# nucypher/TFHE.jl

Measured on AMD Instinct MI355X. Metric: bootstrapped gates/sec (whole node), N=1024, higher is better.
Workload: dtype int32 torus / f64 transform; 1 GPU; batch of 4096 independent gate_nand() bootstraps per GPU, tfhe_parameters_80 (n=500, N=1024, k=1, l=2, Bg=2^10, ks t=8, base 2^2); inputs=resident in HBM, launch=one process

## Files before the change

tfhe.jl_amd/csrc/engine.hpp:

```cpp
#pragma once
#include <hip/hip_runtime.h>

#include <algorithm>
#include <atomic>
#include <cstdarg>
#include <cstdio>
#include <cstring>
#include <new>
#include <string>
#include <thread>
#include <vector>

#include "../../include/tfhe_mi355x.h"
#include "experiment.hpp"
#include "br_core.hpp"

using namespace tfhe;

#include "kernels_blind_rotate.hpp"
#include "kernels_anyn.hpp"
#include "kernels_n512.hpp"
#include "kernels_keyswitch.hpp"

struct ErrBuf {
    char s[512] = {0};
    const char *c_str() const { return s; }
    void set(const char *msg) { snprintf(s, sizeof s, "%s", msg ? msg : ""); }
    ErrBuf &operator=(const char *msg) { set(msg); return *this; }
    void format(const char *fmt, ...) __attribute__((format(printf, 2, 3)))
    {
        va_list ap;
        va_start(ap, fmt);
        vsnprintf(s, sizeof s, fmt, ap);
        va_end(ap);
    }
};
extern thread_local ErrBuf g_create_error;

struct DevBuf {
    void *p = nullptr;
    size_t cap = 0;
    hipError_t reserve(size_t bytes)
    {
        if (bytes <= cap) return hipSuccess;
        if (p) (void)hipFree(p);
        p = nullptr; cap = 0;
        size_t want = bytes + bytes / 4 + 256;
        hipError_t e = hipMalloc(&p, want);
        if (e == hipSuccess) cap = want;
        return e;
    }
    void release() { if (p) (void)hipFree(p); p = nullptr; cap = 0; }
};

struct PairXfer {
    static constexpr int kSlots = 4;
    struct Slot {
        DevBuf out, idx_src;
        DevBuf in, idx_dst;
        int32_t *h_idx = nullptr; size_t h_idx_cap = 0;
        void *h_rows = nullptr; size_t h_rows_cap = 0;
        hipEvent_t ready = nullptr;
        hipEvent_t taken = nullptr;
        bool pending = false;
    } slot[kSlots];
    unsigned next = 0;
};

struct KsKey {
    int mode = 0;
    int parties = 1;
    int kN = 0;
    void *p = nullptr;
    size_t per_party = 0;
    int stride = 0;
    int wtiles = 0;
};
inline void release(KsKey &k)
{
    if (k.p) (void)hipFree(k.p);
    k = KsKey{};
}

struct tfhe_ctx {
    tfhe_params P{};
    int device = 0;
    ErrBuf err;
    std::vector<tfhe_ctx *> kids;
    std::vector<uint8_t> kid_ran;

    hipStream_t stream = nullptr;
    static constexpr int kTimingSlots = 33;
    hipEvent_t evring[kTimingSlots][4] = {};
    hipEvent_t *ev = evring[0];
    int64_t timed_calls = 0;
    hipEvent_t done_ev = nullptr;
    bool done_pending = false;
    bool timing_valid = false;
    bool own_pending = false;
    int64_t last_rotations = 0;
    std::string last_kernel;
    int ks_slices_large = 2;
    int ks_variant = 4;
    int64_t br_small = 1024;
    int br_prio_pct = 90;
    int br_general = 0;
    int br_split = 1;
    int timing_events = 1;
    int br_rt_l = 0;
    int64_t br_tiny = -2;

    cplx *d_tables = nullptr;
    Tables T{};
    Gadget g{};
    cplx *d_anyn_tab = nullptr;
    int br_anyn = 0;
    int anyn_spec = -1;
    bool anyn() const
    {
        if (br_anyn) return true;
        if (P.parties > 1) return P.N != kN || P.parties > 8 || P.bs_l > 8;
        if (n512()) return false;
        return (P.N != kN && P.N != 2048) || P.k > 4;
    }
    bool n512() const { return !br_anyn && P.parties == 1 && P.N == 512 && P.k == 1; }

    cplx *d_bk = nullptr;       size_t bk_polys = 0;
    KsKey ks;
    bool have_bk = false;
    bool have_ks() const { return ks.mode != 0 && ks.parties == 1; }
    cplx *d_mk_bk = nullptr;
    int mk_parties = 0;
    bool have_mk_bk = false;
    bool have_mk_ks() const { return ks.mode != 0 && ks.parties > 1; }

    int32_t *d_wires = nullptr; int64_t num_wires = 0;
    int wires_parties = 0;
    size_t wire_words() const { return wires_parties ? (size_t)wires_parties * P.n + 1 : (size_t)P.n + 1; }

    DevBuf bara, ext, map, io[4], diag, abar, mk_acc, spec;
    DevBuf tv, tv_index;
    DevBuf tv_bodies, tv_ext;
    cplx *d_tgsw = nullptr;        int64_t tgsw_count = 0;
    DevBuf lvl_ws[2], lvl_data, lvl_spec;
    cplx *d_mk_tgsw = nullptr;     int64_t mk_tgsw_count = 0;
    int32_t *d_mk_tgsw_party = nullptr;
    size_t diag_rows = 0;
    bool mk_force_general = false;
    int n2048_rw = 0;
    int mkg_rw = 0;
    int mkg_variant = 0;
    int mkg_acc = -1;
    int mk_rw = 0;
    bool measure_margin = false;
    int exact_domain = 2;
    double exact_bound_log2 = 0;
    double exact_margin = 0;
    tfhe_ctx *twin = nullptr;
    std::atomic<hipStream_t> twin_stream{nullptr};
    bool borrows_keys = false;
    bool slot_busy[2] = {false, false};
    std::atomic<std::thread::id> submit_thread{};
    uint32_t submits = 0;
    std::vector<std::vector<uint8_t>> wire_valid;
    std::vector<int32_t> wire_owner;
    std::vector<uint8_t> peer_ok;
    std::vector<struct PairXfer *> xfer;
    int level_exchange = 0;
    int64_t level_split_min = 4096;
    std::vector<int32_t> kid_tickets[2];
    int cu_count = 256;
    int w2_rw = 0;
    int n512_w2 = -1;
    int n512_rw = 0;
    int k2_w3 = -1;
    int k2_rw = 0;
    int v3_rw = 0;
    int64_t pipeline_min = 4096;
    bool last_call_two_streams = false;
    struct MapStage { void *h = nullptr; size_t cap = 0; hipEvent_t ev = nullptr; bool pending = false; };
    static constexpr int kMapStages = 4;
    MapStage map_stage[kMapStages];
    unsigned map_next = 0;
    MapStage *map_cur = &map_stage[0];
    void *h_map = nullptr;
    hipEvent_t map_ev = nullptr;
// ... 70 lines not shown
constexpr size_t kTan2TableOffset = kN512TableOffset + kN512TableElems;

inline int ilog2i(int x) { int r = 0; while ((1 << r) < x) r++; return r; }
inline bool op_has_a(int op) { return !(op == TFHE_GATE_CONST0 || op == TFHE_GATE_CONST1); }
inline bool op_has_b(int op) { return op_has_a(op) && !(op == TFHE_GATE_NOT || op == TFHE_GATE_COPY); }
inline size_t bk_poly_count(const tfhe_params &p) { return (size_t)p.n * p.bs_l * (p.k + 1) * (p.k + 1); }

template <typename F>
struct ScopeExit {
    F f;
    ~ScopeExit() { f(); }
};
template <typename F>
ScopeExit<F> on_exit(F f) { return ScopeExit<F>{f}; }

template <typename F>
static int32_t fan_out(tfhe_ctx *c, const std::vector<int> &which, F &&fn)
{
    std::vector<int32_t> rcs(which.size(), TFHE_OK);
    std::vector<std::thread> th;
    std::vector<size_t> inline_ones;
    th.reserve(which.size());
    inline_ones.reserve(which.size());
    auto shard = [&](size_t i) noexcept {
        try { rcs[i] = fn(which[i]); } catch (...) { rcs[i] = abi_caught(c->kids[(size_t)which[i]], "fan-out shard"); }
    };
    for (size_t i = 1; i < which.size(); i++) {
        try {
            th.emplace_back([&shard, i] { shard(i); });
        } catch (...) {
            inline_ones.push_back(i);
        }
    }
    if (!which.empty()) shard(0);
    for (size_t i : inline_ones) shard(i);
    for (auto &t : th) t.join();
    std::fill(c->kid_ran.begin(), c->kid_ran.end(), 0);
    for (int k : which) c->kid_ran[(size_t)k] = 1;
    for (size_t i = 0; i < which.size(); i++)
        if (rcs[i]) return c->set_err(rcs[i], "device %d (kid %d): %s", c->kids[(size_t)which[i]]->device, which[i], c->kids[(size_t)which[i]]->err.c_str());
    return TFHE_OK;
}
inline std::vector<int> all_kids(const tfhe_ctx *c)
{
    std::vector<int> v(c->kids.size());
    for (size_t i = 0; i < v.size(); i++) v[i] = (int)i;
    return v;
}

template <typename F>
static int32_t multi_rows(tfhe_ctx *c, int64_t B, F &&call)
{
    const int nk = (int)c->kids.size();
    std::vector<int> which;
    std::vector<int64_t> lo((size_t)nk), hi((size_t)nk);
    for (int r = 0; r < nk; r++) {
        lo[(size_t)r] = B * r / nk; hi[(size_t)r] = B * (r + 1) / nk;
        if (hi[(size_t)r] > lo[(size_t)r]) which.push_back(r);
    }
    return fan_out(c, which, [&](int r) { return call(c->kids[(size_t)r], lo[(size_t)r], hi[(size_t)r] - lo[(size_t)r]); });
}

void shard_bounds_by_rotations(const uint8_t *opcodes, int64_t B, int shards, int64_t *bounds);
void quiesce(tfhe_ctx *c);
int32_t tgsw_prepare(tfhe_ctx *c, const int32_t *d_polys, cplx *d_out, size_t npolys, hipStream_t s);
void mk_tgsw_drop(tfhe_ctx *c);
struct DiagArgs;
int32_t prepare_diag(tfhe_ctx *c, size_t R, hipStream_t s, DiagArgs &d);
void name_kernel(tfhe_ctx *c, const char *fmt, ...) __attribute__((format(printf, 2, 3)));
struct TvPtrs { const int32_t *tv; const int32_t *index; int32_t *bodies = nullptr; int32_t n_out = 1; };
template <class A>
static WithTv<A> with_tv(const A &a, const TvPtrs &tv)
{
    WithTv<A> t;
    static_cast<A &>(t) = a;
    t.tv = tv.tv;
    t.tv_index = tv.index;
    t.bodies = tv.bodies;
    t.n_out = tv.n_out;
    return t;
}
int32_t launch_blind_rotate(tfhe_ctx *c, size_t R, int32_t mu, hipStream_t s, const TvPtrs *tv = nullptr);
int32_t launch_keyswitch(tfhe_ctx *c, size_t G, const int32_t *e0, const int32_t *e1, const int32_t *dst, const int32_t *ext, int32_t *out, hipStream_t s);
int32_t enter_stream(tfhe_ctx *c, hipStream_t s);
int32_t leave_stream(tfhe_ctx *c, hipStream_t s);
void next_timing_slot(tfhe_ctx *c);
void commit_timing_slot(tfhe_ctx *c);
int32_t ensure_host_map(tfhe_ctx *c, size_t bytes);
int32_t launch_prologue(tfhe_ctx *c, size_t R, const int32_t *d_in0, const int32_t *d_in1, const int32_t *d_in2, const int32_t *d_ra, const int32_t *d_rb,
                        const uint8_t *d_kind, int words, hipStream_t s);
int32_t run_gates(tfhe_ctx *c, const char *who, const uint8_t *opcodes, int64_t B, const int32_t *d_in0, const int32_t *d_in1, const int32_t *d_in2,
                  int32_t *d_out, const int32_t *ia, const int32_t *ib, const int32_t *ic, const int32_t *io, hipStream_t s);
int32_t launch_linear_prologue(tfhe_ctx *c, bool lut, size_t B, const int32_t *d_start, const int32_t *d_wire, const int32_t *d_coef,
                               const int32_t *d_cst, const int32_t *d_out, hipStream_t s);
struct IntLevel {
    const int32_t *tv; int32_t n_tv; const int32_t *tv_index; int32_t n_out;
    const int32_t *term_start, *term_wire, *term_coef, *cst, *out;
    int64_t B;
};
int32_t run_int_level(tfhe_ctx *c, const IntLevel &L);
int32_t launch_trivial(tfhe_ctx *c, size_t T, const int32_t *d_in0, const int32_t *d_ts, const int32_t *d_td, const uint8_t *d_top, int32_t *d_out,
                       int words, hipStream_t s);
int32_t launch_mk_blind_rotate(tfhe_ctx *c, size_t R, hipStream_t s, const TvPtrs *tv = nullptr);
int32_t mk_tv_launch_anyn(tfhe_ctx *c, const WithTv<anyn::Args> &a, unsigned nblk, unsigned nt, size_t lds, hipStream_t s);
int32_t mk_tv_launch_w2(tfhe_ctx *c, const WithTv<MkBrArgs> &a, int rw, unsigned nblk, size_t lds, hipStream_t s);
int32_t mk_tv_launch_general(tfhe_ctx *c, const WithTv<MkGenArgs> &a, int rw, bool accg, unsigned nblk, size_t lds, hipStream_t s);
int32_t run_mk_gates(tfhe_ctx *c, const char *who, const uint8_t *opcodes, int64_t B, const int32_t *d_in0, const int32_t *d_in1, const int32_t *d_in2,
                     int32_t *d_out, const int32_t *ia, const int32_t *ib, const int32_t *ic, const int32_t *io, hipStream_t s);
struct BrLaunch {
    int L;
    int rw;
    bool dg;
    dim3 grid, block;
    size_t lds;
};
int32_t br_launch_anyn(tfhe_ctx *c, const WithTv<anyn::Args> &a, const BrLaunch &g, hipStream_t s);
int32_t br_launch_n512w2(tfhe_ctx *c, const WithTv<N512Args> &a, const BrLaunch &g, hipStream_t s);
int32_t br_launch_n512(tfhe_ctx *c, const WithTv<N512Args> &a, const BrLaunch &g, hipStream_t s);
int32_t br_launch_general(tfhe_ctx *c, const WithTv<BrGenArgs> &a, bool n2048, const BrLaunch &g, hipStream_t s);
int32_t br_launch_n2048x(tfhe_ctx *c, const WithTv<Br2048Args> &a, const BrLaunch &g, hipStream_t s);
int32_t br_launch_k2w3(tfhe_ctx *c, const WithTv<BrArgs> &a, const BrLaunch &g, hipStream_t s);
int32_t br_launch_k2(tfhe_ctx *c, const WithTv<BrArgs> &a, const BrLaunch &g, hipStream_t s);
int32_t br_launch_h2(tfhe_ctx *c, const WithTv<BrArgs> &a, const H2Tables &ht, const BrLaunch &g, hipStream_t s);
int32_t br_launch_w2(tfhe_ctx *c, const WithTv<BrArgs> &a, const BrLaunch &g, hipStream_t s);
int32_t br_launch_v3(tfhe_ctx *c, const WithTv<BrArgs> &a, const BrLaunch &g, hipStream_t s);
struct LvlWant { DevBuf *buf; size_t bytes; };
int32_t leveled_reserve(tfhe_ctx *c, const char *who, const LvlWant *want, int count);
int32_t pull_wires(tfhe_ctx *c, int dst, const int32_t *wires, int64_t count);
```

tfhe.jl_amd/csrc/engine_diag.hip:

```cpp
#include "engine.hpp"

int32_t tfhe_last_timing_ms(tfhe_ctx *c, int32_t which, float *ms) try
{
    ENTER_CTX(c);
    if (!c || !ms) return TFHE_ERR_INVALID_ARG;
    if (c->multi()) {
        float worst = -1.f;
        for (size_t k = 0; k < c->kids.size(); k++) {
            if (!c->kid_ran[k]) continue;
            float v = 0.f;
            const int32_t rc = tfhe_last_timing_ms(c->kids[k], which, &v);
            if (rc) { c->err = c->kids[k]->err; return rc; }
            worst = v > worst ? v : worst;
        }
        if (worst < 0.f) return c->set_err(TFHE_ERR_STATE, "last_timing: no batch call recorded");
        *ms = worst;
        return TFHE_OK;
    }
    if (!c->timing_valid) return c->set_err(TFHE_ERR_STATE, "last_timing: no batch call recorded");
    HIP_TRY(c, hipSetDevice(c->device));
    HIP_TRY(c, hipEventSynchronize(c->ev[3]));
    int a, b;
    switch (which) {
    case 0: a = 1; b = 2; break;
// ... 120 lines not shown
        *mhz = f[f.size() / 2];
    }
    return TFHE_OK;
}

int32_t tfhe_last_rounding_margin(tfhe_ctx *c, double *worst) try
{
    ENTER_CTX(c);
    if (!c || !worst) return TFHE_ERR_INVALID_ARG;
    if (c->multi()) {
        double m = -1;
        for (size_t k = 0; k < c->kids.size(); k++) {
            if (!c->kid_ran[k]) continue;
            double v = 0;
            const int32_t rc = read_diag(c->kids[k], &v, nullptr);
            if (rc) { c->err = c->kids[k]->err; return rc; }
            m = v > m ? v : m;
        }
        if (m < 0) return c->set_err(TFHE_ERR_STATE, "last_rounding_margin: no batch call recorded");
        *worst = m;
        return TFHE_OK;
    }
    return read_diag(c, worst, nullptr);
}
ABI_CATCH(c, "tfhe_last_rounding_margin")

int32_t tfhe_last_kernel_clock_mhz(tfhe_ctx *c, double *mhz) try
{
    ENTER_CTX(c);
    if (!c || !mhz) return TFHE_ERR_INVALID_ARG;
    if (c->multi()) {
        for (size_t k = 0; k < c->kids.size(); k++) {
            if (!c->kid_ran[k]) continue;
            const int32_t rc = read_diag(c->kids[k], nullptr, mhz);
            if (rc) c->err = c->kids[k]->err;
            return rc;
        }
        return c->set_err(TFHE_ERR_STATE, "last_kernel_clock: no batch call recorded");
    }
    return read_diag(c, nullptr, mhz);
}
ABI_CATCH(c, "tfhe_last_kernel_clock_mhz")

#ifdef TFHE_STAMP
extern "C" int32_t tfhe_debug_phases(tfhe_ctx *c, unsigned long long *out64)
{
    if (!c || !out64 || c->multi() || !c->diag_rows) return TFHE_ERR_STATE;
    HIP_TRY(c, hipSetDevice(c->device));
    HIP_TRY(c, hipDeviceSynchronize());
    HIP_TRY(c, hipMemcpyAsync(out64, (const char *)c->diag.p + c->diag_rows * 24, 64 * 8, hipMemcpyDeviceToHost, c->stream));
    HIP_TRY(c, hipStreamSynchronize(c->stream));
    return TFHE_OK;
}
#endif

int32_t tfhe_get_option(tfhe_ctx *c, const char *name, int64_t *value) try
{
    if (!c && name && value && !strcmp(name, "debug_fail_alloc_after")) { *value = g_fail_alloc_countdown.load(); return TFHE_OK; }
    ENTER_CTX(c);
    if (!name || !value) return c->set_err(TFHE_ERR_INVALID_ARG, "get_option: NULL argument");
    if (!strcmp(name, "exact_domain")) { *value = c->exact_domain; return TFHE_OK; }
    if (!strcmp(name, "exact_bound_log2_x1000")) { *value = (int64_t)std::llround(c->exact_bound_log2 * 1000.0); return TFHE_OK; }
    if (!strcmp(name, "exact_margin_x1e6")) { *value = (int64_t)std::llround(c->exact_margin * 1e6); return TFHE_OK; }
    if (!strcmp(name, "debug_fail_alloc_after")) { *value = g_fail_alloc_countdown.load(); return TFHE_OK; }
    if (c->multi() && !strcmp(name, "peer_pairs")) {
        int64_t n = 0;
        const size_t nk = c->kids.size();
        for (size_t a = 0; a < nk; a++)
            for (size_t b = 0; b < nk; b++) n += (a != b && c->peer_ok[a * nk + b]) ? 1 : 0;
        *value = n;
        return TFHE_OK;
    }
    if (c->multi() && strcmp(name, "level_split_min") && strcmp(name, "level_exchange")) {
        const int32_t rc = tfhe_get_option(c->kids[0], name, value);
        if (rc) c->err = c->kids[0]->err;
        return rc;
    }
    const struct { const char *n; int64_t v; } table[] = {
        {"br_small", c->br_small}, {"br_tiny", c->br_tiny}, {"br_rt_l", c->br_rt_l}, {"timing_events", c->timing_events},
        {"br_split", c->br_split}, {"br_general", c->br_general}, {"br_anyn", c->br_anyn}, {"anyn_spec", c->anyn_spec},
        {"level_split_min", c->level_split_min}, {"level_exchange", c->level_exchange}, {"br_prio_pct", c->br_prio_pct}, {"ks_slices", c->ks_slices_large},
        {"measure_margin", c->measure_margin ? 1 : 0}, {"pipeline_min", c->pipeline_min}, {"w2_rw", c->w2_rw}, {"k2_rw", c->k2_rw}, {"k2_w3", c->k2_w3}, {"n512_rw", c->n512_rw}, {"n512_w2", c->n512_w2},
        {"v3_rw", c->v3_rw}, {"mk_general", c->mk_force_general ? 1 : 0}, {"n2048_rw", c->n2048_rw}, {"mkg_acc", c->mkg_acc},
        {"mkg_variant", c->mkg_variant}, {"mkg_rw", c->mkg_rw}, {"mk_rw", c->mk_rw}, {"ks_variant", c->ks_variant},
    };
    for (const auto &e : table)
        if (!strcmp(name, e.n)) { *value = e.v; return TFHE_OK; }
    return c->set_err(TFHE_ERR_INVALID_ARG, "get_option: unknown option '%s'", name);
}
ABI_CATCH(c, "tfhe_get_option")

int32_t tfhe_set_option(tfhe_ctx *c, const char *name, int64_t value) try
{
    if (name && !strcmp(name, "debug_fail_alloc_after")) {
        if (value < 0) return TFHE_ERR_INVALID_ARG;
        g_fail_alloc_countdown.store(value);
        return TFHE_OK;
    }
    ENTER_CTX(c);
    if (!c) return TFHE_ERR_INVALID_ARG;
    if (!name || !*name) return TFHE_OK;
    if (c->multi()) {
        if (!strcmp(name, "level_split_min")) { c->level_split_min = value; return TFHE_OK; }
        if (!strcmp(name, "level_exchange")) {
            if (value < 0 || value > 2) return c->set_err(TFHE_ERR_INVALID_ARG, "set_option: level_exchange must be 0 (by peer access), 1 (device-to-device) or 2 (host staging)");
            c->level_exchange = (int)value;
            return TFHE_OK;
        }
        for (tfhe_ctx *k : c->kids) {
            const int32_t rc = tfhe_set_option(k, name, value);
            if (rc) { c->err = k->err; return rc; }
        }
        return TFHE_OK;
    }
    if (!strcmp(name, "br_small")) { c->br_small = value; return TFHE_OK; }
    if (!strcmp(name, "br_tiny")) { c->br_tiny = value; return TFHE_OK; }
    if (!strcmp(name, "br_rt_l")) { c->br_rt_l = value != 0; return TFHE_OK; }
    if (!strcmp(name, "timing_events")) { c->timing_events = value != 0; return TFHE_OK; }
    if (!strcmp(name, "br_split")) { c->br_split = value != 0; return TFHE_OK; }
    if (!strcmp(name, "br_general")) { c->br_general = value != 0; return TFHE_OK; }
    if (!strcmp(name, "br_anyn")) {
        if ((c->have_bk || c->have_mk_bk) && (value != 0) != (c->br_anyn != 0))
            return c->set_err(TFHE_ERR_STATE, "set_option: br_anyn must be chosen before the bootstrapping key is loaded (reload the key after changing it)");
        c->br_anyn = value != 0;
        return TFHE_OK;
    }
    if (!strcmp(name, "anyn_spec")) {
        if (value < -1 || value > 1) return c->set_err(TFHE_ERR_INVALID_ARG, "set_option: anyn_spec must be -1 (LDS when it fits), 0 (LDS) or 1 (global memory)");
        c->anyn_spec = (int)value;
        return TFHE_OK;
    }
    if (!strcmp(name, "level_split_min") || !strcmp(name, "level_exchange")) return TFHE_OK;
    if (!strcmp(name, "br_prio_pct")) {
        if (value < 0 || value > 100) return c->set_err(TFHE_ERR_INVALID_ARG, "set_option: br_prio_pct must be 0..100");
        c->br_prio_pct = (int)value;
        return TFHE_OK;
    }
    if (!strcmp(name, "ks_slices")) {
        if (value != 1 && value != 2 && value != 4) return c->set_err(TFHE_ERR_INVALID_ARG, "set_option: ks_slices must be 1, 2 or 4");
        c->ks_slices_large = (int)value;
        return TFHE_OK;
    }
    if (!strcmp(name, "measure_margin")) { c->measure_margin = value != 0; return TFHE_OK; }
    if (!strcmp(name, "pipeline_min")) { c->pipeline_min = value; return TFHE_OK; }
    if (!strcmp(name, "w2_rw")) {
        if (value < 0 || value > 2) return c->set_err(TFHE_ERR_INVALID_ARG, "set_option: w2_rw must be 0 (by batch size), 1 or 2");
        c->w2_rw = (int)value;
        return TFHE_OK;
    }
    if (!strcmp(name, "n512_w2")) {
        if (value < -1 || value > 1) return c->set_err(TFHE_ERR_INVALID_ARG, "set_option: n512_w2 must be -1 (by batch size), 0 (never) or 1 (always)");
        c->n512_w2 = (int)value;
        return TFHE_OK;
    }
    if (!strcmp(name, "n512_rw")) {
        if (value != 0 && value != 1 && value != 4) return c->set_err(TFHE_ERR_INVALID_ARG, "set_option: n512_rw must be 0 (by batch size), 1 or 4");
        c->n512_rw = (int)value;
        return TFHE_OK;
    }
    if (!strcmp(name, "k2_w3")) {
        if (value < -1 || value > 1) return c->set_err(TFHE_ERR_INVALID_ARG, "set_option: k2_w3 must be -1 (by batch size), 0 (never) or 1 (always)");
        c->k2_w3 = (int)value;
        return TFHE_OK;
    }
    if (!strcmp(name, "k2_rw")) {
        if (value != 0 && value != 1 && value != 7) return c->set_err(TFHE_ERR_INVALID_ARG, "set_option: k2_rw must be 0 (by batch size), 1 or 7");
        c->k2_rw = (int)value;
        return TFHE_OK;
    }
    if (!strcmp(name, "v3_rw")) {
        if (value != 0 && value != 1 && value != 4) return c->set_err(TFHE_ERR_INVALID_ARG, "set_option: v3_rw must be 0 (by batch size), 1 or 4");
        c->v3_rw = (int)value;
        return TFHE_OK;
    }
    if (!strcmp(name, "mk_general")) { c->mk_force_general = value != 0; return TFHE_OK; }
    if (!strcmp(name, "n2048_rw")) {
        if (value != 0 && value != 1 && value != 2) return c->set_err(TFHE_ERR_INVALID_ARG, "set_option: n2048_rw must be 0 (by batch size), 1 or 2");
        c->n2048_rw = (int)value;
        return TFHE_OK;
    }
    if (!strcmp(name, "mkg_acc")) {
        if (value < -1 || value > 1) return c->set_err(TFHE_ERR_INVALID_ARG, "set_option: mkg_acc must be -1 (by party count), 0 (LDS) or 1 (global memory)");
        c->mkg_acc = (int)value;
        return TFHE_OK;
    }
    if (!strcmp(name, "mkg_variant")) {
        if (value != 0 && value != 1) return c->set_err(TFHE_ERR_INVALID_ARG, "set_option: mkg_variant must be 0 (two-wave kernel for the shipped 4- / 8-party sets) or 1 (any-party kernel)");
        c->mkg_variant = (int)value;
        return TFHE_OK;
    }
    if (!strcmp(name, "mkg_rw")) {
        if (value != 0 && value != 1 && value != 2 && value != 4) return c->set_err(TFHE_ERR_INVALID_ARG, "set_option: mkg_rw must be 0 (by batch size), 1, 2 or 4 (4: the two-wave 4- / 8-party kernel only)");
        c->mkg_rw = (int)value;
        return TFHE_OK;
    }
    if (!strcmp(name, "mk_rw")) {
        if (value != 0 && value != 1 && value != 2) return c->set_err(TFHE_ERR_INVALID_ARG, "set_option: mk_rw must be 0 (by batch size), 1 or 2");
        c->mk_rw = (int)value;
        return TFHE_OK;
    }
    if (!strcmp(name, "ks_variant")) {
        if (value != 1 && value != 3 && value != 4) return c->set_err(TFHE_ERR_INVALID_ARG, "set_option: ks_variant must be 1, 3 or 4");
        if (c->ks.mode != 0 && (int)value != c->ks_variant)
            return c->set_err(TFHE_ERR_STATE, "set_option: ks_variant must be chosen before the keyswitch key is loaded (reload the key after changing it)");
        c->ks_variant = (int)value;
        return TFHE_OK;
    }
    return c->set_err(TFHE_ERR_INVALID_ARG, "set_option: unknown option '%s'", name);
}
ABI_CATCH(c, "tfhe_set_option")
```

tfhe.jl_amd/csrc/engine_dispatch.hip:

```cpp
#define TFHE_EMIT_KEYSWITCH_KERNELS
#include "engine.hpp"
#include "br_launch.hpp"

#include <map>
#include <mutex>
#include <functional>

int32_t ensure_dyn_lds(tfhe_ctx *c, const void *fn, size_t bytes, const char *what)
{
    static std::mutex mu;
    static std::map<std::pair<int, const void *>, size_t> have;
    std::lock_guard<std::mutex> lk(mu);
    size_t &cur = have[std::make_pair(c->device, fn)];
    if (cur >= bytes) return TFHE_OK;
    const hipError_t e = hipFuncSetAttribute(fn, hipFuncAttributeMaxDynamicSharedMemorySize, (int)bytes);
    if (e != hipSuccess) return c->set_err(TFHE_ERR_DEVICE, "hipFuncSetAttribute(%s, %zu bytes of LDS) failed: %s", what, bytes, hipGetErrorString(e));
    cur = bytes;
    return TFHE_OK;
}

int32_t prepare_diag(tfhe_ctx *c, size_t R, hipStream_t s, DiagArgs &d)
{
    d.margin_bits = nullptr; d.clk = nullptr; d.phase = nullptr;
    c->diag_rows = 0;
// ... 184 lines not shown
    if (q <= 7 && !allow_w3) return {{R, 0}};
    std::vector<double> best(q + 1, 1e300);
    std::vector<int> take(q + 1, 0);
    best[0] = 0.0;
    for (size_t i = 1; i <= q; i++)
        for (int n = 1; n <= 7 && (size_t)n <= i; n++)
            if (best[i - n] + kK2RoundCost[n] < best[i]) { best[i] = best[i - n] + kK2RoundCost[n]; take[i] = n; }
    int tail = 0;
    double total = best[q];
    for (int t = 1; allow_w3 && t <= 2 && (size_t)t <= q; t++)
        if (best[q - t] + kK2W3RoundCost[t] < total) { total = best[q - t] + kK2W3RoundCost[t]; tail = t; }
    std::vector<int> rounds;
    for (size_t i = q - (size_t)tail; i > 0; i -= (size_t)take[i]) rounds.push_back(take[i]);
    std::sort(rounds.begin(), rounds.end(), std::greater<int>());
    std::vector<K2Seg> seg;
    size_t done = 0;
    for (size_t i = 0; i < rounds.size() && done < R;) {
        size_t j = i;
        while (j < rounds.size() && rounds[j] == rounds[i]) j++;
        const size_t want = (size_t)rounds[i] * (j - i) * cus;
        if ((j == rounds.size() && !tail) || done + want >= R) { seg.push_back({R - done, 0}); done = R; break; }
        seg.push_back({want, 0});
        done += want;
        i = j;
    }
    if (done < R) seg.push_back({R - done, 1});
    return seg;
}

int32_t launch_blind_rotate(tfhe_ctx *c, size_t R, int32_t mu, hipStream_t s, const TvPtrs *tv)
{
    if (tv && c->measure_margin) return c->set_err(TFHE_ERR_STATE, "bootstrap_tv: no DIAG instantiation of the TV kernels (measure_margin is on)");
    DiagArgs diag;
    int32_t rc = prepare_diag(c, R, s, diag);
    if (rc) return rc;
    alloc_checkpoint();
    std::vector<K2Seg> seg;
    const bool tuned_l = c->P.bs_l == 2 || c->P.bs_l == 3;
    if (c->anyn()) {
    } else if (c->br_split && !c->br_general && !c->measure_margin && c->P.N == kN && c->P.k == 2 && tuned_l && (c->k2_rw == 0 || c->k2_rw == 7) && c->k2_w3 != 1) {
        seg = k2_partition(R, (size_t)c->cu_count, c->k2_w3 < 0);
    } else if (c->br_split && !c->br_general && c->P.N == kN && c->P.k == 1 && c->br_small > 0) {
        const size_t resident = 8 * (size_t)c->cu_count;
        if (R > resident && R % resident > 0 && R % resident <= (size_t)c->br_small) seg = {{R - R % resident, -1}, {R % resident, -1}};
    }
    auto part = [&](size_t first, size_t count, int kind) {
        const int32_t r = launch_blind_rotate_part(c, first, count, mu, s, diag, kind, tv);
        if (!r && tv) c->last_kernel += "+tv";
        return r;
    };
    if (seg.empty()) return part(0, R, -1);
    if (seg.size() == 1) return part(0, R, seg[0].kind);
    std::string names;
    size_t first = 0;
    for (const K2Seg &sg : seg) {
        rc = part(first, sg.count, sg.kind);
        if (rc) return rc;
        if (names.empty() || names.substr(names.rfind(" + ") == std::string::npos ? 0 : names.rfind(" + ") + 3) != c->last_kernel)
            names += (names.empty() ? "" : " + ") + c->last_kernel;
        first += sg.count;
    }
    c->last_kernel = names;
    return TFHE_OK;
}

template <class A>
static A ks_args(const tfhe_ctx *c, const int32_t *e0, const int32_t *e1, const int32_t *dst, const int32_t *ext, int32_t *out)
{
    const int P = c->ks.parties, kN = c->ks.kN, n = c->P.n;
    A a{};
    a.ext = ext; a.e0 = e0; a.e1 = e1; a.dst = dst; a.out = out;
    a.n = n; a.kN = kN;
    a.in_stride = P * kN + 1; a.in_off = 0; a.in_b = P * kN; a.out_stride = P * n + 1; a.out_off = 0; a.out_b = P * n;
    return a;
}

int32_t launch_keyswitch(tfhe_ctx *c, size_t G, const int32_t *e0, const int32_t *e1, const int32_t *dst, const int32_t *ext, int32_t *out, hipStream_t s)
{
    const KsKey &K = c->ks;
    const int P = K.parties, kN = K.kN, n = c->P.n;
    if (K.mode == 4) {
        Ks4Args a = ks_args<Ks4Args>(c, e0, e1, dst, ext, out);
        a.G = (int)G; a.wtiles = K.wtiles;
        a.kslices = (P > 1 || kN % 512 != 0) ? 1 : (G <= 512 ? 16 : c->ks_slices_large);
        if (a.kslices > 1) {
            const Ks3Args i3 = ks_args<Ks3Args>(c, e0, e1, dst, ext, out);
            hipLaunchKernelGGL(ks3_init_kernel, dim3((unsigned)G), dim3(256), 0, s, i3);
        }
        a.Gpad = (int)((G + 63) / 64 * 64);
        HIP_TRY(c, c->abar.reserve((size_t)(kN / 4) * a.Gpad * 16));
        a.abar_t = (const i32x4 *)c->abar.p;
        for (int p = 0; p < P; p++) {
            a.in_off = p * kN; a.out_off = p * n; a.add_b = (p == 0);
            a.bmat = (const i32x4 *)K.p + (size_t)p * K.per_party;
            hipLaunchKernelGGL(ks4_digits_kernel, dim3((unsigned)(a.Gpad / 32), (unsigned)(kN / 128)), dim3(128), 0, s, a, (i32x4 *)c->abar.p);
            hipLaunchKernelGGL(keyswitch_kernel_v4, dim3((unsigned)((G + 255) / 256), (unsigned)K.wtiles, (unsigned)a.kslices), dim3(256), 0, s, a);
        }
    } else if (K.mode == 3) {
        Ks3Args a = ks_args<Ks3Args>(c, e0, e1, dst, ext, out);
        a.t = c->P.ks_t; a.log2_base = 2; a.stride = K.stride; a.G = (int)G;
        a.ksp = (const int32_t *)K.p;
        hipLaunchKernelGGL(ks3_init_kernel, dim3((unsigned)G), dim3(256), 0, s, a);
        const unsigned tiles = (unsigned)((G + KS3_G - 1) / KS3_G);
        for (int p = 0; p < P; p++) {
            a.in_off = p * kN; a.out_off = p * n;
            a.ksp = (const int32_t *)K.p + (size_t)p * K.per_party;
            hipLaunchKernelGGL(keyswitch_kernel_v3, dim3(tiles * KS3_SLICES, (unsigned)((K.stride + 511) / 512)), dim3(128), 0, s, a);
        }
    } else {
        KsArgs a = ks_args<KsArgs>(c, e0, e1, dst, ext, out);
        a.t = c->P.ks_t; a.log2_base = c->P.ks_log2_base;
        for (int p = 0; p < P; p++) {
            a.in_off = p * kN; a.out_off = p * n; a.add_b = (p == 0);
            a.ks = (const int32_t *)K.p + (size_t)p * K.per_party;
            hipLaunchKernelGGL(keyswitch_kernel, dim3((unsigned)G, (unsigned)((n + 1 + 256 * KS1_WPT - 1) / (256 * KS1_WPT))), dim3(256), 0, s, a);
        }
    }
    HIP_TRY(c, hipGetLastError());
    return TFHE_OK;
}
```

tfhe.jl_amd/csrc/engine_gates.hip:

```cpp
#include "engine.hpp"
#include <chrono>
#include "kernels_gates.hpp"

int32_t enter_stream(tfhe_ctx *c, hipStream_t s)
{
    if (c->own_pending && s != c->stream) {
        HIP_TRY(c, hipEventRecord(c->done_ev, c->stream));
        c->own_pending = false;
        c->done_pending = true;
    }
    if (!c->done_pending) return TFHE_OK;
    const hipError_t q = hipEventQuery(c->done_ev);
    if (q == hipSuccess) { c->done_pending = false; return TFHE_OK; }
    if (q != hipErrorNotReady) return c->set_err(TFHE_ERR_DEVICE, "hipEventQuery failed: %s", hipGetErrorString(q));
    HIP_TRY(c, hipStreamWaitEvent(s, c->done_ev, 0));
    return TFHE_OK;
}
int32_t leave_stream(tfhe_ctx *c, hipStream_t s)
{
    if (s == c->stream) { c->own_pending = true; return TFHE_OK; }
    c->own_pending = false;
    HIP_TRY(c, hipEventRecord(c->done_ev, s));
    c->done_pending = true;
    return TFHE_OK;
// ... 128 lines not shown
    if (!no_ev) HIP_TRY(c, hipEventRecord(c->ev[3], s));
    if (Tn > 0) {
        hipLaunchKernelGGL(trivial_gates_kernel, dim3((unsigned)Tn), dim3(256), 0, s, d_in0, d_ts, d_td, d_top, d_out, n);
        HIP_TRY(c, hipGetLastError());
    }
    if (!no_ev) commit_timing_slot(c);
    c->last_rotations = (int64_t)R;
    MARK(7);
#ifdef TFHE_EXPERIMENT
    if (dbg_host) fprintf(stderr, "run_gates host us: classify+enter %.0f | stage %.0f | fill %.0f | map H2D %.0f | map event %.0f | prologue %.0f | blind rotate %.0f | keyswitch+trivial %.0f\n",
                          t_acc[0], t_acc[1], t_acc[2], t_acc[3], t_acc[4], t_acc[5], t_acc[6], t_acc[7]);
#endif
    return leave_stream(c, s);
}

int32_t launch_prologue(tfhe_ctx *c, size_t R, const int32_t *d_in0, const int32_t *d_in1, const int32_t *d_in2, const int32_t *d_ra, const int32_t *d_rb,
                        const uint8_t *d_kind, int words, hipStream_t s)
{
    hipLaunchKernelGGL(prologue_kernel, dim3((unsigned)R), dim3(256), 0, s, d_in0, d_in1, d_in2, d_ra, d_rb, d_kind, (int32_t *)c->bara.p, words, ilog2i(2 * c->P.N));
    HIP_TRY(c, hipGetLastError());
    return TFHE_OK;
}

int32_t launch_linear_prologue(tfhe_ctx *c, bool lut, size_t B, const int32_t *d_start, const int32_t *d_wire, const int32_t *d_coef,
                               const int32_t *d_cst, const int32_t *d_out, hipStream_t s)
{
    const int n = (int)c->wire_words() - 1, log2_2N = ilog2i(2 * c->P.N);
    if (lut)
        hipLaunchKernelGGL(linear_prologue_kernel<true>, dim3((unsigned)B), dim3(256), 0, s, (const int32_t *)c->d_wires, d_start, d_wire, d_coef,
                           d_cst, d_out, (int32_t *)c->bara.p, n, log2_2N);
    else
        hipLaunchKernelGGL(linear_prologue_kernel<false>, dim3((unsigned)B), dim3(256), 0, s, (const int32_t *)c->d_wires, d_start, d_wire, d_coef,
                           d_cst, d_out, c->d_wires, n, log2_2N);
    HIP_TRY(c, hipGetLastError());
    return TFHE_OK;
}

int32_t launch_trivial(tfhe_ctx *c, size_t T, const int32_t *d_in0, const int32_t *d_ts, const int32_t *d_td, const uint8_t *d_top, int32_t *d_out,
                       int words, hipStream_t s)
{
    hipLaunchKernelGGL(trivial_gates_kernel, dim3((unsigned)T), dim3(256), 0, s, d_in0, d_ts, d_td, d_top, d_out, words);
    HIP_TRY(c, hipGetLastError());
    return TFHE_OK;
}

int32_t tfhe_gates_batch_dev(tfhe_ctx *c, const uint8_t *opcodes, const int32_t *d_in0, const int32_t *d_in1,
                             const int32_t *d_in2, int32_t *d_out, int64_t B, void *stream) try
{
    ENTER_CTX(c);
    if (!c) return TFHE_ERR_INVALID_ARG;
    if (c->multi()) {
        if (c->kids.size() != 1) return c->set_err(TFHE_ERR_STATE, "gates_batch_dev: device pointers belong to one device; use tfhe_gates_batch on a multi-device context");
        const int32_t rc = tfhe_gates_batch_dev(c->kids[0], opcodes, d_in0, d_in1, d_in2, d_out, B, stream);
        if (rc) c->err = c->kids[0]->err;
        c->kid_ran[0] = 1;
        return rc;
    }
    if (B < 0 || (B > 0 && (!opcodes || !d_out))) return c->set_err(TFHE_ERR_INVALID_ARG, "gates_batch: NULL argument or negative B");
    if (B == 0) { c->timing_valid = false; c->last_rotations = 0; return TFHE_OK; }
    if (B > (int64_t)1 << 30) return c->set_err(TFHE_ERR_INVALID_ARG, "gates_batch: B too large");
    if (c->P.parties != 1) return c->set_err(TFHE_ERR_STATE, "gates_batch: context is multi-key");
    HIP_TRY(c, hipSetDevice(c->device));
    hipStream_t s = stream ? (hipStream_t)stream : c->stream;
    return run_gates(c, "gates_batch", opcodes, B, d_in0, d_in1, d_in2, d_out, nullptr, nullptr, nullptr, nullptr, s);
}
ABI_CATCH(c, "tfhe_gates_batch_dev")

static int32_t gates_batch_one_stream(tfhe_ctx *c, const uint8_t *opcodes, const int32_t *in0, const int32_t *in1, const int32_t *in2,
                                      int32_t *out, int64_t B, const bool (&need)[3]);

static int32_t ensure_twin(tfhe_ctx *c)
{
    if (!c->twin) {
        tfhe_ctx *t = nullptr;
        const int32_t rc = tfhe_ctx_create(&c->P, c->device, &t);
        if (rc) return c->set_err(rc, "gates_batch: second stream context: %s", g_create_error.c_str());
        t->borrows_keys = true;
        t->pipeline_min = -1;
        c->twin = t;
        c->twin_stream.store(t->stream, std::memory_order_release);
    }
    tfhe_ctx *t = c->twin;
    t->d_bk = c->d_bk; t->bk_polys = c->bk_polys; t->have_bk = c->have_bk; t->ks = c->ks;
    t->ks_slices_large = c->ks_slices_large; t->ks_variant = c->ks_variant; t->br_small = c->br_small; t->br_prio_pct = c->br_prio_pct;
    t->br_tiny = c->br_tiny; t->br_rt_l = c->br_rt_l; t->timing_events = c->timing_events; t->br_split = c->br_split; t->br_general = c->br_general; t->n2048_rw = c->n2048_rw; t->v3_rw = c->v3_rw; t->k2_rw = c->k2_rw; t->w2_rw = c->w2_rw;
    t->br_anyn = c->br_anyn; t->anyn_spec = c->anyn_spec; t->k2_w3 = c->k2_w3; t->n512_rw = c->n512_rw; t->n512_w2 = c->n512_w2;
    return TFHE_OK;
}

static int32_t multi_gates_batch(tfhe_ctx *c, const uint8_t *opcodes, const int32_t *in0, const int32_t *in1, const int32_t *in2,
                                 int32_t *out, int64_t B)
{
    const int nk = (int)c->kids.size();
    for (int64_t g = 0; g < B; g++)
        if (opcodes[g] >= TFHE_GATE__COUNT) return c->set_err(TFHE_ERR_INVALID_ARG, "gates_batch: bad opcode %d at gate %lld", opcodes[g], (long long)g);
    alloc_checkpoint();
    std::vector<int64_t> bounds((size_t)nk + 1);
    shard_bounds_by_rotations(opcodes, B, nk, bounds.data());
    std::vector<int> which;
    for (int r = 0; r < nk; r++)
        if (bounds[(size_t)r + 1] > bounds[(size_t)r]) which.push_back(r);
    const size_t n1 = (size_t)c->P.n + 1;
    return fan_out(c, which, [&](int r) {
        const int64_t s0 = bounds[(size_t)r], cnt = bounds[(size_t)r + 1] - s0;
        auto off = [&](const int32_t *p) { return p ? p + (size_t)s0 * n1 : nullptr; };
        return tfhe_gates_batch(c->kids[(size_t)r], opcodes + s0, off(in0), off(in1), off(in2), out + (size_t)s0 * n1, cnt);
    });
}

int32_t tfhe_gates_batch(tfhe_ctx *c, const uint8_t *opcodes, const int32_t *in0, const int32_t *in1,
                         const int32_t *in2, int32_t *out, int64_t B) try
{
    ENTER_CTX(c);
    if (!c) return TFHE_ERR_INVALID_ARG;
    if (B < 0 || (B > 0 && (!opcodes || !out))) return c->set_err(TFHE_ERR_INVALID_ARG, "gates_batch: NULL argument or negative B");
    if (B == 0) return TFHE_OK;
    if (c->multi()) return multi_gates_batch(c, opcodes, in0, in1, in2, out, B);
    HIP_TRY(c, hipSetDevice(c->device));
    bool need[3] = {false, false, false};
    for (int64_t g = 0; g < B; g++) {
        const int op = opcodes[g];
        if (op >= TFHE_GATE__COUNT) return c->set_err(TFHE_ERR_INVALID_ARG, "gates_batch: bad opcode %d at gate %lld", op, (long long)g);
        need[0] = need[0] || op_has_a(op); need[1] = need[1] || op_has_b(op); need[2] = need[2] || op == TFHE_GATE_MUX;
    }
    if ((need[0] && !in0) || (need[1] && !in1) || (need[2] && !in2))
        return c->set_err(TFHE_ERR_INVALID_ARG, "gates_batch: an operand array required by the opcodes is NULL");
    if (c->pipeline_min >= 0 && B >= c->pipeline_min && B >= 2 && !c->borrows_keys && !c->measure_margin && c->P.parties == 1 &&
        c->have_bk && c->have_ks()) {
        int64_t bounds[3];
        shard_bounds_by_rotations(opcodes, B, 2, bounds);
        if (c->P.N == kN && c->P.k == 1 && (c->P.bs_l == 2 || c->P.bs_l == 3) && !c->br_general && !c->anyn()) {
            const int64_t resident = 8 * (int64_t)c->cu_count;
            int64_t total = 0;
            for (int64_t g = 0; g < B; g++) total += opcodes[g] == TFHE_GATE_MUX ? 2 : op_has_b(opcodes[g]) ? 1 : 0;
            const int64_t target = (total / 2 + resident / 2) / resident * resident;
            if (target > 0 && target < total && total % resident != 0) {
                int64_t cum = 0, g = 0;
                while (g < B && cum < target) { cum += opcodes[g] == TFHE_GATE_MUX ? 2 : op_has_b(opcodes[g]) ? 1 : 0; g++; }
                if (cum == target || cum == target + 1) bounds[1] = g;
            }
        }
        if (bounds[1] > 0 && bounds[1] < B) {
            const int32_t rct = ensure_twin(c);
            if (rct) return rct;
            const size_t n1 = (size_t)c->P.n + 1;
            auto off = [&](const int32_t *p, int64_t g) { return p ? p + (size_t)g * n1 : nullptr; };
            const int64_t h = bounds[1];
            int32_t rc1 = TFHE_OK;
            std::thread second;
            try {
                second = std::thread([&] {
                    try { rc1 = gates_batch_one_stream(c->twin, opcodes + h, off(in0, h), off(in1, h), off(in2, h), out + (size_t)h * n1, B - h, need); }
                    catch (...) { rc1 = abi_caught(c->twin, "gates_batch (second half)"); }
                });
            } catch (const std::exception &) {
                return gates_batch_one_stream(c, opcodes, in0, in1, in2, out, B, need);
            }
            int32_t rc0;
            {
                auto joined = on_exit([&] { second.join(); });
                rc0 = gates_batch_one_stream(c, opcodes, in0, in1, in2, out, h, need);
            }
            if (rc1) return c->set_err(rc1, "gates_batch (second half): %s", c->twin->err.c_str());
            if (rc0) return rc0;
            c->last_rotations += c->twin->last_rotations;
            c->last_call_two_streams = true;
            return TFHE_OK;
// ... 414 lines not shown
```

Measured before the change: 363,500 gates/s.

## Add sparse-MFMA keyswitch path using one-hot digit indices for single-key batches

Adds a keyswitch path that encodes each 2-bit decomposition digit of the extracted LWE mask as a sparsity index word. The key matrix is then multiplied with the AMD sparse int8 MFMA (smfmac 32x32x64) against a constant one-hot operand, replacing the dense keyswitch-v4 product. A separate kernel computes and transposes the digit indices. The main kernel double-buffers key tiles through LDS and can split the reduction across two waves-groups per block with an LDS exchange. It is enabled by default for single-party batches above 512 samples, aiming to cut keyswitch MAC work and bandwidth. It adds an extra launch and relies on correct sparse-index semantics.

Result: no change. 362,800 gates/s (-0.2%).

```diff
diff --git a/tfhe.jl_amd/csrc/engine.hpp b/tfhe.jl_amd/csrc/engine.hpp
--- a/tfhe.jl_amd/csrc/engine.hpp
+++ b/tfhe.jl_amd/csrc/engine.hpp
@@ -102,6 +102,7 @@
     std::string last_kernel;
     int ks_slices_large = 2;
     int ks_variant = 4;
+    int ks_sparse = 1;
     int64_t br_small = 1024;
     int br_prio_pct = 90;
     int br_general = 0;
@@ -338,6 +339,7 @@
 }
 int32_t launch_blind_rotate(tfhe_ctx *c, size_t R, int32_t mu, hipStream_t s, const TvPtrs *tv = nullptr);
 int32_t launch_keyswitch(tfhe_ctx *c, size_t G, const int32_t *e0, const int32_t *e1, const int32_t *dst, const int32_t *ext, int32_t *out, hipStream_t s);
+int32_t launch_keyswitch_sparse(tfhe_ctx *c, const Ks4Args &a, int ks, hipStream_t s);
 int32_t enter_stream(tfhe_ctx *c, hipStream_t s);
 int32_t leave_stream(tfhe_ctx *c, hipStream_t s);
 void next_timing_slot(tfhe_ctx *c);
diff --git a/tfhe.jl_amd/csrc/engine_diag.hip b/tfhe.jl_amd/csrc/engine_diag.hip
--- a/tfhe.jl_amd/csrc/engine_diag.hip
+++ b/tfhe.jl_amd/csrc/engine_diag.hip
@@ -226,7 +226,7 @@
         {"level_split_min", c->level_split_min}, {"level_exchange", c->level_exchange}, {"br_prio_pct", c->br_prio_pct}, {"ks_slices", c->ks_slices_large},
         {"measure_margin", c->measure_margin ? 1 : 0}, {"pipeline_min", c->pipeline_min}, {"w2_rw", c->w2_rw}, {"k2_rw", c->k2_rw}, {"k2_w3", c->k2_w3}, {"n512_rw", c->n512_rw}, {"n512_w2", c->n512_w2},
         {"v3_rw", c->v3_rw}, {"mk_general", c->mk_force_general ? 1 : 0}, {"n2048_rw", c->n2048_rw}, {"mkg_acc", c->mkg_acc},
-        {"mkg_variant", c->mkg_variant}, {"mkg_rw", c->mkg_rw}, {"mk_rw", c->mk_rw}, {"ks_variant", c->ks_variant},
+        {"mkg_variant", c->mkg_variant}, {"mkg_rw", c->mkg_rw}, {"mk_rw", c->mk_rw}, {"ks_variant", c->ks_variant}, {"ks_sparse", c->ks_sparse},
     };
     for (const auto &e : table)
         if (!strcmp(name, e.n)) { *value = e.v; return TFHE_OK; }
@@ -285,6 +285,11 @@
         c->ks_slices_large = (int)value;
         return TFHE_OK;
     }
+    if (!strcmp(name, "ks_sparse")) {
+        if (value < 0 || value > 2) return c->set_err(TFHE_ERR_INVALID_ARG, "set_option: ks_sparse must be 0 (never), 1 (single-key batches above 512 samples) or 2 (every single-key batch)");
+        c->ks_sparse = (int)value;
+        return TFHE_OK;
+    }
     if (!strcmp(name, "measure_margin")) { c->measure_margin = value != 0; return TFHE_OK; }
     if (!strcmp(name, "pipeline_min")) { c->pipeline_min = value; return TFHE_OK; }
     if (!strcmp(name, "w2_rw")) {
diff --git a/tfhe.jl_amd/csrc/engine_dispatch.hip b/tfhe.jl_amd/csrc/engine_dispatch.hip
--- a/tfhe.jl_amd/csrc/engine_dispatch.hip
+++ b/tfhe.jl_amd/csrc/engine_dispatch.hip
@@ -290,7 +290,9 @@
     if (K.mode == 4) {
         Ks4Args a = ks_args<Ks4Args>(c, e0, e1, dst, ext, out);
         a.G = (int)G; a.wtiles = K.wtiles;
-        a.kslices = (P > 1 || kN % 512 != 0) ? 1 : (G <= 512 ? 16 : c->ks_slices_large);
+        const bool sparse = P == 1 && kN % 512 == 0 && (c->ks_sparse == 2 || (c->ks_sparse == 1 && G > 512));
+        if (sparse) a.kslices = c->ks_slices_large == 4 ? 2 : 1;
+        else a.kslices = (P > 1 || kN % 512 != 0) ? 1 : (G <= 512 ? 16 : c->ks_slices_large);
         if (a.kslices > 1) {
             const Ks3Args i3 = ks_args<Ks3Args>(c, e0, e1, dst, ext, out);
             hipLaunchKernelGGL(ks3_init_kernel, dim3((unsigned)G), dim3(256), 0, s, i3);
@@ -298,6 +300,11 @@
         a.Gpad = (int)((G + 63) / 64 * 64);
         HIP_TRY(c, c->abar.reserve((size_t)(kN / 4) * a.Gpad * 16));
         a.abar_t = (const i32x4 *)c->abar.p;
+        if (sparse) {
+            a.add_b = 1;
+            a.bmat = (const i32x4 *)K.p;
+            return launch_keyswitch_sparse(c, a, c->ks_slices_large >= 2 ? 2 : 1, s);
+        }
         for (int p = 0; p < P; p++) {
             a.in_off = p * kN; a.out_off = p * n; a.add_b = (p == 0);
             a.bmat = (const i32x4 *)K.p + (size_t)p * K.per_party;
diff --git a/tfhe.jl_amd/csrc/engine_gates.hip b/tfhe.jl_amd/csrc/engine_gates.hip
--- a/tfhe.jl_amd/csrc/engine_gates.hip
+++ b/tfhe.jl_amd/csrc/engine_gates.hip
@@ -234,7 +234,7 @@
     }
     tfhe_ctx *t = c->twin;
     t->d_bk = c->d_bk; t->bk_polys = c->bk_polys; t->have_bk = c->have_bk; t->ks = c->ks;
-    t->ks_slices_large = c->ks_slices_large; t->ks_variant = c->ks_variant; t->br_small = c->br_small; t->br_prio_pct = c->br_prio_pct;
+    t->ks_slices_large = c->ks_slices_large; t->ks_variant = c->ks_variant; t->ks_sparse = c->ks_sparse; t->br_small = c->br_small; t->br_prio_pct = c->br_prio_pct;
     t->br_tiny = c->br_tiny; t->br_rt_l = c->br_rt_l; t->timing_events = c->timing_events; t->br_split = c->br_split; t->br_general = c->br_general; t->n2048_rw = c->n2048_rw; t->v3_rw = c->v3_rw; t->k2_rw = c->k2_rw; t->w2_rw = c->w2_rw;
     t->br_anyn = c->br_anyn; t->anyn_spec = c->anyn_spec; t->k2_w3 = c->k2_w3; t->n512_rw = c->n512_rw; t->n512_w2 = c->n512_w2;
     return TFHE_OK;
diff --git a/tfhe.jl_amd/csrc/engine_keyswitch.hip b/tfhe.jl_amd/csrc/engine_keyswitch.hip
--- /dev/null
+++ b/tfhe.jl_amd/csrc/engine_keyswitch.hip
@@ -0,0 +1,17 @@
+#define TFHE_EMIT_KEYSWITCH_SPARSE_KERNELS
+#include "engine.hpp"
+#include "kernels_keyswitch_sparse.hpp"
+
+int32_t launch_keyswitch_sparse(tfhe_ctx *c, const Ks4Args &a, int ks, hipStream_t s)
+{
+    KsSparseArgs S{};
+    S.k = a;
+    S.idx_t = (const i32x2 *)c->abar.p;
+    S.xblocks = (a.G + 255) / 256;
+    hipLaunchKernelGGL(ks_sparse_digits_kernel, dim3((unsigned)(a.Gpad / 32), (unsigned)(a.kN / 128)), dim3(128), 0, s, a, (i32x2 *)c->abar.p);
+    const dim3 grid((unsigned)(a.wtiles * S.xblocks), 1, (unsigned)a.kslices);
+    if (ks == 2) hipLaunchKernelGGL(keyswitch_kernel_sparse<2>, grid, dim3(512), 0, s, S);
+    else hipLaunchKernelGGL(keyswitch_kernel_sparse<1>, grid, dim3(256), 0, s, S);
+    HIP_TRY(c, hipGetLastError());
+    return TFHE_OK;
+}
diff --git a/tfhe.jl_amd/csrc/kernels_keyswitch_sparse.hpp b/tfhe.jl_amd/csrc/kernels_keyswitch_sparse.hpp
--- /dev/null
+++ b/tfhe.jl_amd/csrc/kernels_keyswitch_sparse.hpp
@@ -0,0 +1,175 @@
+#pragma once
+#include <hip/hip_runtime.h>
+
+#include "kernels_keyswitch.hpp"
+
+typedef int32_t i32x2 __attribute__((ext_vector_type(2)));
+typedef int32_t i32x8 __attribute__((ext_vector_type(8)));
+
+struct KsSparseArgs {
+    Ks4Args k;
+    const i32x2 *idx_t;
+    int32_t xblocks;
+};
+
+__host__ __device__ inline uint32_t ks_sparse_index_word(uint32_t abar)
+{
+    uint32_t idx = 0;
+#pragma unroll
+    for (int g = 0; g < 8; g++) {
+        const uint32_t d = (abar >> (30 - 2 * g)) & 3u;
+        idx |= (d | ((d ^ 1u) << 2)) << (4 * g);
+    }
+    return idx;
+}
+
+#ifdef TFHE_EMIT_KEYSWITCH_SPARSE_KERNELS
+__global__ __launch_bounds__(128) void ks_sparse_digits_kernel(Ks4Args P, i32x2 *__restrict__ idx_t)
+{
+    __shared__ uint32_t tile[32][129];
+    const int tid = threadIdx.x;
+    const int g0 = blockIdx.x * 32, i0 = blockIdx.y * 128;
+    for (int g = 0; g < 32; g++) {
+        const int gg = min(g0 + g, P.G - 1);
+        const int32_t *r0 = P.ext + (size_t)P.e0[gg] * P.in_stride + P.in_off;
+        const int e1 = P.e1 ? P.e1[gg] : -1;
+        uint32_t v = (uint32_t)r0[i0 + tid];
+        if (e1 >= 0) v += (uint32_t)P.ext[(size_t)e1 * P.in_stride + P.in_off + i0 + tid];
+        tile[g][tid] = ks_sparse_index_word(v + (1u << 15));
+    }
+    __syncthreads();
+    for (int k = tid; k < 32 * 2 * 32; k += 128) {
+        const int q = k >> 6, h = (k >> 5) & 1, g = k & 31;
+        i32x2 o;
+        o[0] = (int32_t)tile[g][4 * q + h];
+        o[1] = (int32_t)tile[g][4 * q + 2 + h];
+        idx_t[((size_t)(i0 / 4 + q) * 2 + h) * P.Gpad + g0 + g] = o;
+    }
+}
+
+template <int KS>
+__global__ __launch_bounds__(256 * KS, KS == 1 ? 2 : 1) void keyswitch_kernel_sparse(KsSparseArgs S)
+{
+    constexpr int MT = 2;
+    const Ks4Args &P = S.k;
+    __shared__ i32x4 bst[KS][2][4][4][64];
+    const int lane = threadIdx.x & 63, wave = (threadIdx.x >> 6) & 3, ksl = threadIdx.x >> 8;
+    const int c = lane & 31, h = lane >> 5;
+    const int wt = (int)blockIdx.x / S.xblocks;
+    const int gbase = (((int)blockIdx.x % S.xblocks) * 4 + wave) * (32 * MT);
+    const bool wave_active = gbase < P.G;
+
+    const i32x2 *ip[MT];
+#pragma unroll
+    for (int mt = 0; mt < MT; mt++) ip[mt] = S.idx_t + (size_t)h * P.Gpad + min(gbase + mt * 32 + c, P.Gpad - 1);
+
+    i32x16 acc[MT][4];
+#pragma unroll
+    for (int mt = 0; mt < MT; mt++)
+#pragma unroll
+        for (int pl = 0; pl < 4; pl++)
+#pragma unroll
+            for (int r = 0; r < 16; r++) acc[mt][pl][r] = 0;
+
+    const size_t bstep = (size_t)P.wtiles * 4 * 64;
+    const int span = P.kN / ((int)gridDim.z * KS);
+    const int i_begin = ((int)blockIdx.z * KS + ksl) * span;
+    const i32x4 *bp = P.bmat + (size_t)i_begin * bstep + ((size_t)wt * 4 + wave) * 64 + lane;
+    const int stages = span / 4;
+    auto load_b = [&](int st, i32x4 (&r)[4]) {
+        const int sc = min(st, stages - 1);
+#pragma unroll
+        for (int ii = 0; ii < 4; ii++) r[ii] = bp[(size_t)(4 * sc + ii) * bstep];
+    };
+    auto store_b = [&](int buf, const i32x4 (&r)[4]) {
+#pragma unroll
+        for (int ii = 0; ii < 4; ii++) bst[ksl][buf][ii][wave][lane] = r[ii];
+    };
+    auto load_a = [&](int st, i32x2 (&a)[MT]) {
+        const int sc = min(st, stages - 1);
+#pragma unroll
+        for (int mt = 0; mt < MT; mt++) a[mt] = ip[mt][(size_t)(i_begin / 4 + sc) * 2 * P.Gpad];
+    };
+    const i32x4 one_hot = {0x00010001, 0x00010001, 0x00010001, 0x00010001};
+    auto compute = [&](int buf, const i32x2 (&a)[MT]) {
+        if (!wave_active) return;
+#pragma unroll
+        for (int pr = 0; pr < 2; pr++)
+#pragma unroll
+            for (int pl = 0; pl < 4; pl++) {
+                const i32x4 b0 = bst[ksl][buf][2 * pr][pl][lane], b1 = bst[ksl][buf][2 * pr + 1][pl][lane];
+                const i32x8 bfrag = {b0[0], b0[1], b0[2], b0[3], b1[0], b1[1], b1[2], b1[3]};
+#pragma unroll
+                for (int mt = 0; mt < MT; mt++)
+                    acc[mt][pl] = __builtin_amdgcn_smfmac_i32_32x32x64_i8(one_hot, bfrag, acc[mt][pl], a[mt][pr], 0, 0);
+            }
+    };
+
+    i32x4 pre_e[4], pre_o[4];
+    i32x2 a_e[MT], a_o[MT];
+    load_b(0, pre_e);
+    load_b(1, pre_o);
+    load_a(0, a_e);
+    load_a(1, a_o);
+    store_b(0, pre_e);
+    for (int st = 0; st < stages; st += 2) {
+        load_b(st + 2, pre_e);
+        __syncthreads();
+        compute(0, a_e);
+        store_b(1, pre_o);
+        load_a(st + 2, a_e);
+        load_b(st + 3, pre_o);
+        __syncthreads();
+        compute(1, a_o);
+        store_b(0, pre_e);
+        load_a(st + 3, a_o);
+    }
+
+    uint32_t sum[MT][16];
+#pragma unroll
+    for (int mt = 0; mt < MT; mt++)
+#pragma unroll
+        for (int r = 0; r < 16; r++)
+            sum[mt][r] = (uint32_t)acc[mt][0][r] + ((uint32_t)acc[mt][1][r] << 8) + ((uint32_t)acc[mt][2][r] << 16) + ((uint32_t)acc[mt][3][r] << 24);
+    if (KS > 1) {
+        uint32_t *xch = reinterpret_cast<uint32_t *>(&bst[0][0][0][0][0]);
+        __syncthreads();
+        if (ksl > 0)
+#pragma unroll
+            for (int mt = 0; mt < MT; mt++)
+#pragma unroll
+                for (int r = 0; r < 16; r++) xch[(((ksl - 1) * 4 + wave) * (MT * 16) + mt * 16 + r) * 64 + lane] = sum[mt][r];
+        __syncthreads();
+        if (ksl > 0) return;
+        for (int k = 1; k < KS; k++)
+#pragma unroll
+            for (int mt = 0; mt < MT; mt++)
+#pragma unroll
+                for (int r = 0; r < 16; r++) sum[mt][r] += xch[(((k - 1) * 4 + wave) * (MT * 16) + mt * 16 + r) * 64 + lane];
+    }
+    if (!wave_active) return;
+
+    const int w = wt * 32 + c;
+    if (w > P.n) return;
+#pragma unroll
+    for (int mt = 0; mt < MT; mt++)
+#pragma unroll
+        for (int r = 0; r < 16; r++) {
+            const int gg = gbase + mt * 32 + (r & 3) + 8 * (r >> 2) + 4 * h;
+            if (gg >= P.G) continue;
+            const uint32_t s = sum[mt][r];
+            const size_t og = P.dst ? (size_t)P.dst[gg] : (size_t)gg;
+            int32_t *o = P.out + og * P.out_stride;
+            if (gridDim.z > 1) {
+                atomicAdd(reinterpret_cast<unsigned int *>(o + (w < P.n ? P.out_off + w : P.out_b)), 0u - s);
+            } else if (w < P.n) {
+                o[P.out_off + w] = (int32_t)(0u - s);
+            } else {
+                uint32_t b = (uint32_t)P.ext[(size_t)P.e0[gg] * P.in_stride + P.in_b];
+                const int e1 = P.e1 ? P.e1[gg] : -1;
+                if (e1 >= 0) b += (uint32_t)P.ext[(size_t)e1 * P.in_stride + P.in_b] + (1u << 29);
+                o[P.out_b] = (int32_t)(b - s);
+            }
+        }
+}
+#endif
```
